# darnstrom/daqp

Measured on AMD Instinct MI355X. Metric: QPs/sec (fp64) for batched random dense QPs n=50 m=150, higher is better.
Workload: dtype f64; 1 GPU; C2: 100000 random dense QPs per GPU, n=50 m=150 ms=0, 20 active at the optimum; batch_per_gpu=100000, parallelism=1 rank(s), shards only, no data-path collective

## Files before the change

daqp_amd/_lib.py:

```python
import ctypes as C
import os
import shutil
import subprocess

PKG = os.path.dirname(os.path.abspath(__file__))
ROOT = os.path.dirname(PKG)
CSRC = os.path.join(PKG, "csrc")
LIBDIR = os.path.join(PKG, "lib")
LIBPATH = os.path.join(LIBDIR, "libdaqp_amd.so")

c_double_p = C.POINTER(C.c_double)
c_int_p = C.POINTER(C.c_int)


class DAQPSettings(C.Structure):
    _fields_ = [("primal_tol", C.c_double), ("dual_tol", C.c_double), ("zero_tol", C.c_double),
                ("pivot_tol", C.c_double), ("progress_tol", C.c_double),
                ("cycle_tol", C.c_int), ("iter_limit", C.c_int),
                ("fval_bound", C.c_double), ("eps_prox", C.c_double), ("eta_prox", C.c_double),
                ("rho_soft", C.c_double), ("rel_subopt", C.c_double), ("abs_subopt", C.c_double),
                ("sing_tol", C.c_double), ("refactor_tol", C.c_double), ("time_limit", C.c_double)]


class DAQPProblem(C.Structure):
# ... 3 lines not shown
                ("break_points", c_int_p), ("nh", C.c_int), ("problem_type", C.c_int)]


class DAQPResult(C.Structure):
    _fields_ = [("x", c_double_p), ("lam", c_double_p), ("fval", C.c_double), ("soft_slack", C.c_double),
                ("exitflag", C.c_int), ("iter", C.c_int), ("nodes", C.c_int),
                ("solve_time", C.c_double), ("setup_time", C.c_double)]


class DAQPBatchProblem(C.Structure):
    _fields_ = [("N", C.c_int), ("n", C.c_int), ("m", C.c_int), ("ms", C.c_int),
                ("H", C.c_void_p), ("f", C.c_void_p), ("A", C.c_void_p),
                ("bupper", C.c_void_p), ("blower", C.c_void_p), ("sense", C.c_void_p),
                ("memory", C.c_int)]


class DAQPBatchResult(C.Structure):
    _fields_ = [("x", C.c_void_p), ("lam", C.c_void_p), ("fval", C.c_void_p), ("soft_slack", C.c_void_p),
                ("exitflag", C.c_void_p), ("iter", C.c_void_p), ("memory", C.c_int),
                ("setup_time", C.c_double), ("solve_time", C.c_double)]


WORKSPACE_BYTES = 288
MEM_HOST, MEM_DEVICE = 0, 1

EXPORTS = [
    "daqp_quadprog", "daqp_solve", "setup_daqp", "setup_daqp_main", "daqp_update_ldp", "daqp_default_settings",
    "allocate_daqp_settings", "free_daqp_workspace", "free_daqp_ldp", "daqp_primal_init_active",
    "daqp_dual_init_active", "daqp_set_primal_start", "daqp_minrep", "allocate_daqp_workspace", "allocate_daqp_ldp", "daqp_first_violating", "daqp_batch_create", "daqp_batch_free", "daqp_amd_release_pool", "daqp_amd_shutdown", "daqp_batch_set_stream",
    "daqp_batch_set_settings", "daqp_batch_set_exact", "daqp_batch_setup", "daqp_batch_setup_shared", "daqp_batch_update", "daqp_batch_solve",
    "daqp_batch_setup_flags", "daqp_batch_working_sets", "daqp_batch_set_primal_start", "daqp_batch_prox_info", "daqp_quadprog_batch", "daqp_quadprog_batch_multi", "daqp_batch_kernel_ms",
    "daqp_batch_create_multi", "daqp_batch_free_multi", "daqp_batch_multi_shards", "daqp_batch_multi_shard", "daqp_batch_setup_multi", "daqp_batch_update_multi",
    "daqp_batch_solve_multi", "daqp_batch_setup_multi_shards", "daqp_batch_update_multi_shards", "daqp_batch_solve_multi_shards",
    "daqp_batch_device_bytes", "daqp_batch_rechecked", "daqp_batch_set_recheck", "daqp_batch_recheck_ms", "daqp_amd_last_error", "daqp_amd_device_count", "daqp_amd_version", "daqp_amd_has_tiny",
    "setup_daqp_ldp", "daqp_ldp", "ldp2qp_solution", "daqp_extract_result",
    "daqp_minrep_batch", "daqp_minrep_batch_info", "daqp_batch_reset", "reset_daqp_workspace", "daqp_deactivate_constraints",
    "daqp_batch_backward",
    "daqp_batch_enable_trace", "daqp_batch_read_trace", "daqp_batch_enable_profile", "daqp_batch_read_profile", "daqp_batch_read_ldp",
]


UNITS = {
    "daqp_amd.hip": ["daqp_amd.hip", "kernels.hip.h", "wave_ldp.hip.h", "wave_ldp_reg.hip.h", "setup_fast.hip.h", "prox.hip.h",
                     "wg_layout.hip.h", "batch_dev.hip.h", "recheck.hip.h", "minrep.hip.h", "backward.hip.h", "setup_m.hip.h", "setup_fact.hip.h", "reg_kernel.hip.h", "tiny_setup.hip.h", "setup_blk.hip.h", "multi.hip.h"],
    "reg_kernel.hip": ["reg_kernel.hip", "reg_kernel.hip.h", "wave_ldp_reg.hip.h", "wave_ldp.hip.h", "batch_dev.hip.h"],
    "reg32_kernel.hip": ["reg32_kernel.hip", "reg_kernel.hip.h", "wave_ldp_reg.hip.h", "wave_ldp.hip.h", "batch_dev.hip.h"],
    "wg_kernel.hip": ["wg_kernel.hip", "wg_kernel.hip.h", "wg_ldp.hip.h", "wg_layout.hip.h", "batch_dev.hip.h", "wave_ldp.hip.h", "wave_ldp_reg.hip.h"],
    "backward_kernel.hip": ["backward_kernel.hip", "backward.hip.h", "batch_dev.hip.h", "wave_ldp.hip.h"],
    "setup_kernel.hip": ["setup_kernel.hip", "setup_blk.hip.h", "setup_fast.hip.h", "setup_m.hip.h", "setup_fact.hip.h", "tiny_setup.hip.h", "wave_ldp_reg.hip.h", "wave_ldp.hip.h", "batch_dev.hip.h"],
}
HIPFLAGS = ["--offload-arch=gfx950", "-O3", "-std=c++17", "-ffp-contract=off", "-fPIC"]
OBJDIR = os.path.join(LIBDIR, "obj")
UNITS = {u: d for u, d in UNITS.items() if os.path.exists(os.path.join(CSRC, u))}


def units(extra_flags=()):
    return list(UNITS)


def _flag_key(extra_flags=()):
    return " ".join([*HIPFLAGS, *extra_flags])


def _unit_stale(unit, extra_flags=()):
    obj = os.path.join(OBJDIR, unit + ".o")
    if not os.path.exists(obj) or not os.path.exists(obj + ".resources.txt"):
        return True
# ... 85 lines not shown
        cur = None
        with open(path) as fh:
            for line in fh:
                m = re.search(r"remark:\s+Function Name: (\S+)", line)
                if m:
                    cur = out.setdefault(m.group(1), {})
                    continue
                m = re.search(r"remark:\s+([A-Za-z][^:]*): (\d+)", line)
                if m and cur is not None and m.group(1) in keys:
                    cur[keys[m.group(1)]] = int(m.group(2))
    try:
        names = subprocess.run(["c++filt"], input="\n".join(out), capture_output=True, text=True, check=True).stdout.split("\n")
        out = {n.replace("daqp_amd::", "").split("(")[0].replace("void ", ""): v for n, v in zip(names, out.values())}
    except (OSError, subprocess.CalledProcessError):
        pass
    return out


_lib = None


def lib():
    global _lib
    if _lib is not None:
        return _lib
    if not os.path.exists(LIBPATH):
        build()
    L = C.CDLL(os.environ.get("DAQP_AMD_LIBRARY") or LIBPATH)
    vp, ci = C.c_void_p, C.c_int
    L.daqp_amd_last_error.restype = C.c_char_p
    L.daqp_amd_version.restype = C.c_char_p
    L.daqp_batch_create.argtypes = [C.POINTER(vp), ci, ci, ci, ci, ci, C.POINTER(DAQPSettings), ci]
    L.daqp_batch_free.argtypes = [vp]
    L.daqp_batch_free.restype = None
    L.daqp_amd_release_pool.argtypes = []
    L.daqp_amd_release_pool.restype = None
    L.daqp_batch_set_stream.argtypes = [vp, vp]
    L.daqp_batch_set_stream.restype = None
    L.daqp_batch_set_settings.argtypes = [vp, C.POINTER(DAQPSettings)]
    L.daqp_batch_set_settings.restype = None
    L.daqp_batch_set_exact.argtypes = [vp, ci]
    L.daqp_batch_set_exact.restype = None
    L.daqp_batch_setup.argtypes = [vp, C.POINTER(DAQPBatchProblem), ci]
    L.daqp_batch_setup_shared.argtypes = [vp, C.POINTER(DAQPBatchProblem), ci]
    L.daqp_batch_update.argtypes = [vp, ci, C.POINTER(DAQPBatchProblem)]
    L.daqp_batch_solve.argtypes = [vp, C.POINTER(DAQPBatchResult)]
    L.daqp_batch_setup_flags.argtypes = [vp, c_int_p]
    L.daqp_batch_working_sets.argtypes = [vp, c_int_p, c_int_p]
    L.daqp_batch_set_primal_start.argtypes = [vp, C.c_void_p, ci]
    L.daqp_batch_prox_info.argtypes = [vp, c_int_p, c_int_p, C.c_void_p]
    L.daqp_quadprog_batch.argtypes = [C.POINTER(DAQPBatchResult), C.POINTER(DAQPBatchProblem), C.POINTER(DAQPSettings)]
    L.daqp_quadprog_batch_multi.argtypes = [C.POINTER(DAQPBatchResult), C.POINTER(DAQPBatchProblem), C.POINTER(DAQPSettings), c_int_p, ci]
    L.daqp_batch_create_multi.argtypes = [C.POINTER(vp), ci, ci, ci, ci, ci, C.POINTER(DAQPSettings), c_int_p, ci]
    L.daqp_batch_free_multi.argtypes = [vp]
    L.daqp_batch_free_multi.restype = None
    L.daqp_batch_multi_shards.argtypes = [vp]
    L.daqp_batch_multi_shard.argtypes = [vp, ci, c_int_p, c_int_p]
    L.daqp_batch_multi_shard.restype = vp
    L.daqp_batch_setup_multi.argtypes = [vp, C.POINTER(DAQPBatchProblem), ci]
    L.daqp_batch_update_multi.argtypes = [vp, ci, C.POINTER(DAQPBatchProblem)]
    L.daqp_batch_solve_multi.argtypes = [vp, C.POINTER(DAQPBatchResult)]
    L.daqp_batch_setup_multi_shards.argtypes = [vp, C.POINTER(DAQPBatchProblem), ci]
    L.daqp_batch_update_multi_shards.argtypes = [vp, ci, C.POINTER(DAQPBatchProblem)]
    L.daqp_batch_solve_multi_shards.argtypes = [vp, C.POINTER(DAQPBatchResult)]
    L.daqp_batch_kernel_ms.argtypes = [vp, C.POINTER(C.c_float), C.POINTER(C.c_float)]
    L.daqp_batch_rechecked.argtypes = [vp]
# ... 60 lines not shown
```

daqp_amd/csrc/daqp_amd.hip:

```cpp
#include <hip/hip_runtime.h>

#include <sched.h>

#include <chrono>
#include <cstdarg>
#include <cstdio>
#include <cstdlib>
#include <cstring>
#include <mutex>
#include <atomic>
#include <vector>
#include <string>
#include <thread>

#include "kernels.hip.h"
#include "reg_kernel.hip.h"
#include "setup_fast.hip.h"
#include "prox.hip.h"
#include "recheck.hip.h"
#include "setup_m.hip.h"
#include "setup_fact.hip.h"
#include "wg_layout.hip.h"
#include "tiny_setup.hip.h"
#include "setup_blk.hip.h"
// ... 757 lines not shown
    return k;
}
void destroy_batch(DAQPBatch *b)
{
    (void)hipSetDevice(b->device);
    (void)hipStreamSynchronize(b->stream);
    if (b->redo) { b->redo->stream = nullptr; destroy_batch(b->redo); b->redo = nullptr; }
    if (b->pin_redo) (void)hipHostFree(b->pin_redo);
    if (b->img_ho_pin) (void)hipHostFree(b->img_ho_pin);
    for (void *p : b->owned) (void)hipFree(p);
    if (b->pin_in) (void)hipHostFree(b->pin_in);
    if (b->pin_out) (void)hipHostFree(b->pin_out);
    if (b->pin_mir) (void)hipHostFree(b->pin_mir);
    if (b->pin_sig) (void)hipHostFree(b->pin_sig);
    if (b->pin_upd) (void)hipHostFree(b->pin_upd);
    if (b->ev_in) (void)hipEventDestroy(b->ev_in);
    if (b->ev_count) (void)hipEventDestroy(b->ev_count);
    if (b->pin_count) (void)hipHostFree(b->pin_count);
    for (auto &e : b->ev) if (e) (void)hipEventDestroy(e);
    for (auto &e : b->ev_r) if (e) (void)hipEventDestroy(e);
    delete b;
}
}

extern "C" {

const char *daqp_amd_last_error(void) { return g_err; }
#ifdef DAQP_AMD_FEW_VARIANTS
const char *daqp_amd_version(void) { return "daqp_amd 0.4 (gfx950, fp64: one wavefront per QP, one workgroup per QP beyond 64 working-set rows, up to 512 rows) [dev build: few template instantiations]"; }
#else
const char *daqp_amd_version(void) { return "daqp_amd 0.4 (gfx950, fp64: one wavefront per QP, one workgroup per QP beyond 64 working-set rows, up to 512 rows)"; }
#endif
int daqp_amd_has_tiny(void) { return 0; }
int daqp_amd_device_count(void)
{
    int c = 0;
    if (hipGetDeviceCount(&c) != hipSuccess) return 0;
    return c;
}
void daqp_default_settings(DAQPSettings *settings) { default_settings(settings); }

static int batch_create(DAQPBatch **out, int N, int n, int m, int ms, int ns_max, const DAQPSettings *settings, int device, int group);
int daqp_batch_create(DAQPBatch **out, int N, int n, int m, int ms, int ns_max, const DAQPSettings *settings, int device)
{
    return batch_create(out, N, n, m, ms, ns_max, settings, device, 0);
}
static int batch_create(DAQPBatch **out, int N, int n, int m, int ms, int ns_max, const DAQPSettings *settings, int device, int group)
{
    if (!out) return DAQP_EXIT_UNSUPPORTED;
    *out = nullptr;
    if (N <= 0 || n <= 0 || m < 0 || ms < 0 || ms > m || ms > n || ns_max < 0) {
        set_err("bad dimensions N=%d n=%d m=%d ms=%d ns=%d", N, n, m, ms, ns_max);
        return DAQP_EXIT_UNSUPPORTED;
    }
    const int cap = n + ns_max + 1;
    if (cap > 512 || n > 511) { set_err("n + ns + 1 = %d exceeds the 512-row working-set limit of this build", cap); return DAQP_EXIT_UNSUPPORTED; }
    int ndev = 0;
    const hipError_t dev_rc = hipGetDeviceCount(&ndev);
    if (dev_rc == hipSuccess && ndev > 0 && device >= 0 && device < 64) {
        static std::once_flag once;
        std::call_once(once, [] { if (!getenv("DAQP_AMD_NO_EXIT_SYNC")) atexit(daqp_amd_shutdown); });
        g_devices_used.fetch_or(1ull << device);
    }
    if (dev_rc != hipSuccess || ndev == 0) {
        set_err("no HIP device: libdaqp_amd has no CPU path");
        return DAQP_EXIT_UNSUPPORTED;
// ... 481 lines not shown
        if (p->sense) { memcpy(hp + o, p->sense, nb * sizeof(int)); d.sense_in = reinterpret_cast<const int *>(dp + o); }
        else d.sense_in = nullptr;
        HIPCHK(hipMemcpyAsync(b->dev_in, b->pin_in, bytes, hipMemcpyHostToDevice, b->stream));
        HIPCHK(hipEventRecord(b->ev_in, b->stream));
    } else {
        rc |= stage(b, p->f, p->memory, N * d.n, &b->sf, &b->nf, &d.f);
        rc |= stage(b, p->A, p->memory, N * d.mA * d.n, &b->sA, &b->nA, &d.A);
        rc |= stage(b, p->bupper, p->memory, N * d.m, &b->sbu, &b->nbu, &d.bu);
        rc |= stage(b, p->blower, p->memory, N * d.m, &b->sbl, &b->nbl, &d.bl);
        rc |= stage(b, p->sense, p->memory, N * d.m, &b->ssense, &b->nsense, &d.sense_in);
    }
    if (rc) return DAQP_EXIT_UNSUPPORTED;
    b->was_shared = false;
    const int mask = (init_mask & ~DAQP_UPDATE_eliminate) | DAQP_UPDATE_Rinv | DAQP_UPDATE_M | DAQP_UPDATE_v | DAQP_UPDATE_d | DAQP_UPDATE_sense;
    setup_kernel_t ks = b->setup_spill ? (d.n > 256 ? k_setup<true, 8> : k_setup<true>) : k_setup<false>;
    size_t lds_setup = b->lds_setup;
    if (b->fast_setup) {
        ks = pick_setup_fast(d.n, d.exact_setup == 0);
        lds_setup = (size_t)fast_lds(d.n, d.m, d.exact_setup, d.mA).total_bytes;
    }
    HIPCHK(hipFuncSetAttribute(reinterpret_cast<const void *>(ks), hipFuncAttributeMaxDynamicSharedMemorySize, (int)lds_setup));
    if (!b->quiet_setup) HIPCHK(hipEventRecord(b->ev[0], b->stream));
    b->inputs_adopted = p->memory == DAQP_MEM_DEVICE;
    if (!lp && b->tiny_setup) {
        hipLaunchKernelGGL(k_setup_tiny<4>, dim3((d.N + 15) / 16), dim3(64), 0, b->stream, d, mask);
        HIPCHK(hipGetLastError());
    } else if (!lp && b->fast_setup && (d.ms == 0 || !getenv("DAQP_AMD_NO_BLK_BOUNDS")) && d.n > 16 && d.exact_setup == 0 && blk_setup_enabled()) {
        const int NT = (d.n + 15) / 16;
        ldp_reg_kernel_t kb = nullptr;
#define DAQP_BLK_SHAPE(nt, nw, tail) \
        if (!kb && NT == nt && d.n <= nw && (tail) == (d.n - 16 * (nt - 1) <= 4)) kb = k_setup_blk<nt, nw, tail>;
        DAQP_BLK_SHAPES
#undef DAQP_BLK_SHAPE
        const size_t lds_blk = (size_t)(NT == 2 ? blk_lds<2>(d.n, d.m) : (NT == 3 ? blk_lds<3>(d.n, d.m) : blk_lds<4>(d.n, d.m))).total_bytes;
        HIPCHK(hipFuncSetAttribute(reinterpret_cast<const void *>(kb), hipFuncAttributeMaxDynamicSharedMemorySize, (int)lds_blk));
        if (push_descriptor(b)) return DAQP_EXIT_UNSUPPORTED;
        hipLaunchKernelGGL(kb, dim3(d.N), dim3(64), lds_blk, b->stream, (const BatchDev *)b->d_dev, mask);
        HIPCHK(hipGetLastError());
        hipLaunchKernelGGL(ks, dim3(d.N), dim3(64), lds_setup, b->stream, d, mask | kSetupOnlyMarked);
        HIPCHK(hipGetLastError());
    } else if (!lp) {
        BatchDev l = d;
        l.defer_m = defers_m(b, d) ? 1 : 0;
        const bool gs_now = b->setup_spill || (b->fact_gs && l.defer_m && b->fact_buf && d.setup_g && !(d.st.eps_prox > 0.0));
        if (l.defer_m) {
            ks = gs_now ? k_setup<true, 4, true> : k_setup<false, 4, true>;
            if (gs_now && !b->setup_spill) lds_setup = (size_t)setup_lds(d.n, d.m, true).total_bytes;
            HIPCHK(hipFuncSetAttribute(reinterpret_cast<const void *>(ks), hipFuncAttributeMaxDynamicSharedMemorySize, (int)lds_setup));
        }
        l.fact = nullptr;
        if (l.defer_m && gs_now && b->fact_buf && d.n <= kFactMaxN && !(d.st.eps_prox > 0.0)) {
            const size_t lds = fact_lds_bytes(d.n);
            if (hipFuncSetAttribute(reinterpret_cast<const void *>(k_fact_wg), hipFuncAttributeMaxDynamicSharedMemorySize, (int)lds) == hipSuccess) {
                l.fact = b->fact_buf;
                hipLaunchKernelGGL(k_fact_wg, dim3(d.N), dim3(512), lds, b->stream, l);
                HIPCHK(hipGetLastError());
            } else (void)hipGetLastError();
        }
        hipLaunchKernelGGL(ks, dim3(d.N), dim3(64), lds_setup, b->stream, l, mask);
        HIPCHK(hipGetLastError());
        if (l.defer_m) { if (launch_setup_m(b, l)) return DAQP_EXIT_UNSUPPORTED; }
    } else HIPCHK(hipMemsetAsync(d.qs, 0, (size_t)d.N * sizeof(QState), b->stream));
    b->reg_pending = false;
    if (b->lean && !lp) {
        b->n_prox_qps = 0;
    } else {
    rc = lp ? regularise(b, d, mask, true) : count_flagged_async(b, mask);
// ... 1013 lines not shown
```

daqp_amd/csrc/setup_blk.hip.h:

```cpp
#pragma once
#include "wave_ldp_reg.hip.h"
#include "batch_dev.hip.h"
#include "setup_fast.hip.h"

namespace daqp_amd {

typedef double blk_v4d __attribute__((ext_vector_type(4)));
typedef double blk_v2d __attribute__((ext_vector_type(2)));
#define BLK_GLOBAL(T) DAQP_GLOBAL(T)
template <class T> __device__ __forceinline__ auto blk_g(T *p) { return as_global(p); }

template <int NT> __host__ __device__ constexpr int blk_tix(int I, int J) { return I * NT - I * (I - 1) / 2 + (J - I); }
constexpr int kBlkScratch = 16 * 17;

template <int K> __device__ __forceinline__ double blk_bcast(double v) { return __builtin_amdgcn_update_dpp(0.0, v, 0x150 + K, 0xf, 0xf, true); }
__device__ __forceinline__ double blk_sum16(double v)
{
    v += dpp_f64<0xB1>(v);
    v += dpp_f64<0x4E>(v);
    v += dpp_f64<0x141>(v);
    v += dpp_f64<0x140>(v);
    return v;
}

template <int NT> __host__ __device__ constexpr int blk_scratch_doubles() { return (NT * (NT - 1) / 2 + NT - 1) * kBlkScratch; }

template <int NT>
__device__ __forceinline__ void blk_load(const double *Hs, int n, double zero_tol, blk_v4d (&T)[NT * (NT + 1) / 2], int &offd)
{
    const int lane = lane_id(), lr = lane & 15, lk = lane >> 4;
    offd = 0;
    static_for<NT>([&](auto Ic) __attribute__((always_inline)) {
        static_for<NT>([&](auto Jc) __attribute__((always_inline)) {
            constexpr int I = Ic, J = Jc;
            if constexpr (I <= J) {
#pragma unroll
                for (int r = 0; r < 4; ++r) {
                    const int i = 16 * I + lk + 4 * r, j = 16 * J + lr;
                    const bool in = i < n && j < n;
                    const double hij = Hs[in ? i * n + j : 0], hji = Hs[in ? j * n + i : 0];
                    if (in && j > i && (hij > zero_tol || hij < -zero_tol)) offd = 1;
                    T[blk_tix<NT>(I, J)][r] = in ? ((i == j) ? hij : 0.5 * (hij + hji)) : ((i == j) ? 1.0 : 0.0);
                }
            }
        });
    });
}

template <int NT>
__device__ __forceinline__ bool blk_factor(blk_v4d (&T)[NT * (NT + 1) / 2], int n, double zero_tol, blk_v4d (&X)[NT * (NT + 1) / 2], double *scr, double &pmin, double &pmax)
{
    const int lane = lane_id(), lr = lane & 15, lk = lane >> 4;
    blk_v4d V[NT];
    double dmin = DAQP_INF, dmax = 0.0, dsum = 0.0;
    static_for<NT>([&](auto Kc) __attribute__((always_inline)) {
        constexpr int K = Kc;
        double c[16];
        {
            const blk_v4d d = T[blk_tix<NT>(K, K)];
#pragma unroll
            for (int r = 0; r < 4; ++r)
#pragma unroll
                for (int g = 0; g < 4; ++g) c[4 * r + g] = __shfl(d[r], 16 * g + lr);
        }
        static_for<16>([&](auto kc) __attribute__((always_inline)) {
            constexpr int k = kc;
            const double d = blk_bcast<k>(c[k]);
            const bool real = 16 * K + k < n;
            dmin = fmin(dmin, real ? d : (double)DAQP_INF);
            dmax = fmax(dmax, real ? d : 0.0);
            dsum += d;
            const double inv = rsqrt(d);
            c[k] = (lr == k) ? inv : c[k] * inv;
            static_for<15 - k>([&](auto ii) __attribute__((always_inline)) {
                constexpr int i = k + 1 + ii;
                c[i] = __builtin_fma(-blk_bcast<i>(c[k]), c[k], c[i]);
            });
        });
// ... 17 lines not shown
                asm volatile("" : "+v"(x0), "+v"(x1), "+v"(x2), "+v"(x3));
                double v = x0;
                v = (lk == 1) ? x1 : v;
                v = (lk == 2) ? x2 : v;
                v = (lk == 3) ? x3 : v;
                V[K][r] = v;
            }
        }
        static_for<NT>([&](auto Jc) __attribute__((always_inline)) {
            constexpr int J = Jc;
            if constexpr (J > K) {
                blk_v4d acc = (blk_v4d){0.0, 0.0, 0.0, 0.0};
                const blk_v4d h = T[blk_tix<NT>(K, J)];
#pragma unroll
                for (int s = 0; s < 4; ++s) acc = __builtin_amdgcn_mfma_f64_16x16x4f64(V[K][s], h[s], acc, 0, 0, 0);
                T[blk_tix<NT>(K, J)] = acc;
            }
        });
        static_for<NT>([&](auto Ic) __attribute__((always_inline)) {
            static_for<NT>([&](auto Jc) __attribute__((always_inline)) {
                constexpr int I = Ic, J = Jc;
                if constexpr (I > K && J >= I) {
                    blk_v4d acc = T[blk_tix<NT>(I, J)];
                    const blk_v4d a = T[blk_tix<NT>(K, I)], bb = T[blk_tix<NT>(K, J)];
#pragma unroll
                    for (int s = 0; s < 4; ++s) acc = __builtin_amdgcn_mfma_f64_16x16x4f64(-a[s], bb[s], acc, 0, 0, 0);
                    T[blk_tix<NT>(I, J)] = acc;
                }
            });
        });
    });
    blk_v4d VT[NT > 1 ? NT - 1 : 1];
    if constexpr (NT > 1) {
        WSYNC();
        static_for<NT>([&](auto Ic) __attribute__((always_inline)) {
            static_for<NT>([&](auto Jc) __attribute__((always_inline)) {
                constexpr int I = Ic, J = Jc;
                if constexpr (I < J) {
                    double *sc = scr + (blk_tix<NT>(I, J) - I - 1) * kBlkScratch;
#pragma unroll
                    for (int r = 0; r < 4; ++r) sc[(lk + 4 * r) * 17 + lr] = T[blk_tix<NT>(I, J)][r];
                }
            });
            if constexpr (Ic < NT - 1) {
                double *sc = scr + (NT * (NT - 1) / 2 + Ic) * kBlkScratch;
#pragma unroll
                for (int r = 0; r < 4; ++r) sc[(lk + 4 * r) * 17 + lr] = V[Ic][r];
            }
        });
        WSYNC();
        static_for<NT>([&](auto Ic) __attribute__((always_inline)) {
            static_for<NT>([&](auto Jc) __attribute__((always_inline)) {
                constexpr int I = Ic, J = Jc;
                if constexpr (I < J) {
                    const double *sc = scr + (blk_tix<NT>(I, J) - I - 1) * kBlkScratch;
#pragma unroll
                    for (int s_ = 0; s_ < 4; ++s_) T[blk_tix<NT>(I, J)][s_] = sc[lr * 17 + 4 * s_ + lk];
                }
            });
            if constexpr (Ic < NT - 1) {
                const double *sc = scr + (NT * (NT - 1) / 2 + Ic) * kBlkScratch;
#pragma unroll
                for (int s_ = 0; s_ < 4; ++s_) VT[Ic][s_] = sc[lr * 17 + 4 * s_ + lk];
            }
        });
    }
    static_for<NT>([&](auto Jc) __attribute__((always_inline)) {
        constexpr int J = Jc;
        X[blk_tix<NT>(J, J)] = V[J];
        static_for<J>([&](auto Ii) __attribute__((always_inline)) {
            constexpr int I = J - 1 - Ii;
            blk_v4d s4 = (blk_v4d){0.0, 0.0, 0.0, 0.0};
            static_for<J - I>([&](auto Kk) __attribute__((always_inline)) {
                constexpr int K = I + 1 + Kk;
                const blk_v4d at = T[blk_tix<NT>(I, K)], xb = X[blk_tix<NT>(K, J)];
#pragma unroll
                for (int s_ = 0; s_ < 4; ++s_) s4 = __builtin_amdgcn_mfma_f64_16x16x4f64(at[s_], xb[s_], s4, 0, 0, 0);
            });
            blk_v4d o4 = (blk_v4d){0.0, 0.0, 0.0, 0.0};
#pragma unroll
            for (int s_ = 0; s_ < 4; ++s_) o4 = __builtin_amdgcn_mfma_f64_16x16x4f64(-VT[I][s_], s4[s_], o4, 0, 0, 0);
            X[blk_tix<NT>(I, J)] = o4;
        });
    });
    pmin = rl(dmin, 0); pmax = rl(dmax, 0);
    const double ds0 = rl(dsum, 0);
    const bool ok = (ds0 == ds0) && (pmin > 2.0 * zero_tol);
    return ok;
}

__host__ __device__ inline int blk_region(int n, int scratch) { const int h = n * n + 8; return h > scratch ? h : scratch; }
__host__ __device__ inline int blk_tile_rows(int n, int scratch)
{
    const int ldr = n | 1;
    int tr = 64;
    while (tr > 16 && tr * ldr > blk_region(n, scratch)) tr -= 16;
    return tr;
}
struct BlkLds { int R, fv, vv, xu, sens, total_bytes; };
template <int NT>
__host__ __device__ inline BlkLds blk_lds(int n, int m)
{
    BlkLds s;
    const int ldr = n | 1, TR = blk_tile_rows(n, blk_scratch_doubles<NT>());
    int r0 = blk_region(n, blk_scratch_doubles<NT>());
    if (r0 < TR * ldr) r0 = TR * ldr;
    int o = round_up(r0, 2);
    s.R = 0;
    s.fv = o; o += 64; s.vv = o; o += 64; s.xu = o; o += 64;
    s.sens = o;
    s.total_bytes = o * 8 + round_up(m, 4) * 4;
    return s;
}

template <int NT, int NW = 16 * NT, bool TAIL = false>
__global__ __launch_bounds__(64) __attribute__((amdgpu_waves_per_eu(2, 2))) void k_setup_blk(const BatchDev *__restrict__ bp, int mask)
{
    extern __shared__ __attribute__((aligned(16))) double smem[];
    static_assert(NW <= 16 * NT && NW > 16 * (NT - 1) && NW % 8 == 0, "column width within the last block");
    static_assert(!TAIL || (NT > 1 && NW == 16 * (NT - 1) + 8), "tail columns: the first eight of the last block");
    constexpr int NTT = NT * (NT + 1) / 2, KT = TAIL ? 4 * (NT - 1) + 1 : NW / 4, CT = TAIL ? NT - 1 : NT;
    const BatchDev &b = *bp;
    const int q = blockIdx.x, lane = lane_id(), lr = lane & 15, lk = lane >> 4;
    const int n = b.n, m = b.m, mA = b.mA, ms = b.ms;
    const BlkLds o = blk_lds<NT>(n, m);
    const int TR = blk_tile_rows(n, blk_scratch_doubles<NT>());
    double *Hs = smem + o.R, *fl = smem + o.fv, *vv = smem + o.vv, *xu = smem + o.xu, *tile = smem + o.R;
    double *srow = fl, *drow = vv;
    const int tailc = TAIL ? n - 16 * (NT - 1) : 0;
    int *sens = reinterpret_cast<int *>(smem + o.sens);
    const double *H = b.H + (size_t)q * n * n, *A = b.A + (size_t)q * mA * n;
    BLK_GLOBAL(QState) *qs = blk_g(b.qs + q);
    const double zero_tol = b.st.zero_tol, primal_tol = b.st.primal_tol;
    const bool force = b.st.eps_prox > 0.0;
    const bool direct = !(n & 1) && (n & 31) && !(((size_t)H | (size_t)A) & 15);
    const int ldr = direct ? n : (n | 1);
    int flag = 1, activate = 0;
    long long pt[10] = {0, 0, 0, 0, 0, 0, 0, 0, 0, 0};
    long long t0 = (kProfile && b.prof) ? (long long)__builtin_readcyclecounter() : 0;
#define SPROF(slot) do { if (kProfile && b.prof) { const long long t1 = (long long)__builtin_readcyclecounter(); pt[slot] += t1 - t0; t0 = t1; } } while (0)

    if (direct) copy_async(Hs, H, n * n);
    {
        const BLK_GLOBAL(double) *bu = blk_g(b.bu + (size_t)q * m), *bl = blk_g(b.bl + (size_t)q * m);
        const BLK_GLOBAL(int) *sin = b.sense_in ? blk_g(b.sense_in + (size_t)q * m) : nullptr;
        int bad = 0;
        for (int i = lane; i < m; i += 64) {
            int s = sin ? sin[i] : 0;
            if (s & DAQP_BINARY) bad |= 2;
            if (!(s & DAQP_IMMUTABLE)) {
                const double diff = bu[i] - bl[i];
                if (diff < -primal_tol) bad |= 1;
                else if (diff < zero_tol && !(s & DAQP_SOFT)) { s |= DAQP_ACTIVE + DAQP_IMMUTABLE; bad |= 4; }
            }
            sens[i] = s;
        }
        bad = (__any(bad & 2) ? 2 : 0) | (__any(bad & 1) ? 1 : 0) | (__any(bad & 4) ? 4 : 0);
        if (b.sense_in) activate = 1;
        if (bad & 4) activate = 1;
        if (bad & 2) flag = DAQP_EXIT_UNSUPPORTED;
        else if (bad & 1) flag = DAQP_EXIT_INFEASIBLE;
        if (force && flag > 0) flag = DAQP_NEEDS_SHIFT;
        fl[lane] = (lane < n) ? blk_g(b.f)[(size_t)q * n + lane] : 0.0;
    }
    int diag = 0;
    blk_v4d X[NTT];
    if (flag > 0) {
        if (direct) copy_wait(); else stage_rows(Hs, H, n, n, n);
        WSYNC();
        blk_v4d T[NTT];
        int offd;
        blk_load<NT>(Hs, n, zero_tol, T, offd);
        SPROF(9);
        if (!__any(offd) && ms > 0) flag = DAQP_NEEDS_ORDERED;
        else if (!__any(offd)) {
            const double hd = (lane < n) ? Hs[lane * n + lane] : 1.0;
            const double ha = hd < 0 ? -hd : hd;
            const double hscale = -wave_min((lane < n) ? -ha : 0.0);
            const double ftol = hscale > 0 ? zero_tol * hscale : zero_tol;
            const bool fail = lane < n && hd <= ftol;
            const int code = (b.st.eps_prox == 0.0 && hd <= zero_tol) ? DAQP_EXIT_NONCONVEX : DAQP_NEEDS_SHIFT;
            const unsigned long long fm = __ballot(fail);
            if (fm) flag = __builtin_amdgcn_readlane(code, __ffsll((long long)fm) - 1);
            else {
                WSYNC();
                xu[lane] = 1 / sqrt(hd);
                WSYNC();
                static_for<NT>([&](auto Ic) __attribute__((always_inline)) {
                    static_for<NT>([&](auto Jc) __attribute__((always_inline)) {
                        constexpr int I = Ic, J = Jc;
                        if constexpr (I <= J) {
#pragma unroll
                            for (int r = 0; r < 4; ++r) X[blk_tix<NT>(I, J)][r] = (I == J && lk + 4 * r == lr) ? xu[16 * I + lr] : 0.0;
                        }
                    });
                });
                diag = 1;
            }
            WSYNC();
        } else {
            WSYNC();
            double pmin = DAQP_INF, pmax = 0.0;
            const bool ok = blk_factor<NT>(T, n, zero_tol, X, Hs, pmin, pmax);
            if (!ok || !(pmin > 2.0 * zero_tol * pmax)) flag = DAQP_NEEDS_ORDERED;
            WSYNC();
        }
    }
    if (flag == DAQP_NEEDS_ORDERED) { if (lane == 0) qs->setup_flag = DAQP_NEEDS_ORDERED; return; }
    SPROF(0);
    int unc = 0;
    double vcol[NT];
    static_for<NT>([&](auto Jc) __attribute__((always_inline)) { vcol[Jc] = 0.0; });
    if (flag > 0) {
        static_for<NT>([&](auto Jc) __attribute__((always_inline)) {
            constexpr int J = Jc;
            double p = 0;
            static_for<J + 1>([&](auto Ic) __attribute__((always_inline)) {
#pragma unroll
                for (int r = 0; r < 4; ++r) p = __builtin_fma(X[blk_tix<NT>(Ic, J)][r], fl[16 * Ic + lk + 4 * r], p);
            });
            p += __shfl_xor(p, 16);
            p += __shfl_xor(p, 32);
            vcol[J] = p;
            if (lk == 0 && 16 * J + lr < n) blk_g(b.v)[(size_t)q * n + 16 * J + lr] = p;
        });
        SPROF(1);
        if (mask & DAQP_UPDATE_unconstrained) {
            int fixed = 0;
            for (int i = lane; i < m; i += 64) fixed |= sens[i] & (DAQP_ACTIVE + DAQP_IMMUTABLE);
            if (!__any(fixed)) {
                unc = 1;
                static_for<NT>([&](auto Ic) __attribute__((always_inline)) {
                    constexpr int I = Ic;
#pragma unroll
                    for (int r = 0; r < 4; ++r) {
                        double p = 0;
                        static_for<NT - I>([&](auto Jj) __attribute__((always_inline)) { p = __builtin_fma(X[blk_tix<NT>(I, I + Jj)][r], vcol[I + Jj], p); });
                        p = blk_sum16(p);
                        if (lr == 0) xu[16 * I + lk + 4 * r] = -p;
                    }
                });
// ... 210 lines not shown
#pragma unroll
                            for (int u = 0; u < 8; ++u) dst[(size_t)((tq + u < npair) ? tq + u : npair - 1) * 64] = (blk_v2d){v8[u].x * scal, v8[u].y * scal};
                        }
                    } else {
                        for (int tq = 0; tq < npair; tq += 8) {
                            double vx[8], vy[8];
#pragma unroll
                            for (int u = 0; u < 8; ++u) {
                                const int t = (tq + u < npair) ? tq + u : npair - 1;
                                vx[u] = a[2 * t];
                                const double y = a[(2 * t + 1 < n) ? 2 * t + 1 : 2 * t];
                                vy[u] = (2 * t + 1 < n) ? y : 0.0;
                            }
#pragma unroll
                            for (int u = 0; u < 8; ++u) dst[(size_t)((tq + u < npair) ? tq + u : npair - 1) * 64] = (blk_v2d){vx[u] * scal, vy[u] * scal};
                        }
                    }
                }
            }
            if (direct && tb + TR < mA) {
                WSYNC();
                copy_async(tile, A + (size_t)(tb + TR) * n, ((mA - tb - TR) < TR ? (mA - tb - TR) : TR) * n);
            }
            if (__any(rowbad)) flag = DAQP_EXIT_INFEASIBLE;
            SPROF(4);
        }
    }
    const int all_feasible = __all(feasible);
    int sing = kEmpty;
    if (flag > 0 && unc && all_feasible) { sing = DAQP_UNCONSTRAINED_OPTIMAL; activate = 0; }
    if (flag > 0) {
        if (lane < n && unc) blk_g(b.xunc)[(size_t)q * n + lane] = xu[lane];
    }
    for (int i = lane; i < m; i += 64) blk_g(b.sense)[(size_t)q * m + i] = sens[i];
    SPROF(5);
    if (lane == 0) {
        qs->n_active = 0; qs->reuse_ind = 0; qs->sing_ind = sing; qs->iterations = 0;
        qs->lam_swapped = 0; qs->setup_flag = flag; qs->need_activate = (flag > 0) ? activate : 0; qs->pad_ = 0;
        qs->exitflag = flag; qs->fval = 0; qs->soft_slack = 0; qs->diag_h = diag; qs->n_prox = 0;
        qs->upd_flag = 0;
        if (kProfile && b.prof) for (int i = 0; i < 10; ++i) blk_g(b.prof)[(size_t)q * 32 + i] = pt[i];
    }
#undef SPROF
}

#define DAQP_BLK_SHAPES \
    DAQP_BLK_SHAPE(2, 24, true) DAQP_BLK_SHAPE(2, 32, false) DAQP_BLK_SHAPE(3, 40, true) DAQP_BLK_SHAPE(3, 48, false) \
    DAQP_BLK_SHAPE(4, 56, true) DAQP_BLK_SHAPE(4, 56, false) DAQP_BLK_SHAPE(4, 64, false)

}
```

include/daqp_amd.h:

```cpp
#ifndef DAQP_AMD_H
#define DAQP_AMD_H

#ifdef __cplusplus
extern "C" {
#endif

typedef double c_float;

#define DAQP_EXIT_SOFT_OPTIMAL 2
#define DAQP_EXIT_OPTIMAL 1
#define DAQP_EXIT_INFEASIBLE -1
#define DAQP_EXIT_CYCLE -2
#define DAQP_EXIT_UNBOUNDED -3
#define DAQP_EXIT_ITERLIMIT -4
#define DAQP_EXIT_NONCONVEX -5
#define DAQP_EXIT_OVERDETERMINED_INITIAL -6
#define DAQP_EXIT_TIMELIMIT -7
#define DAQP_EXIT_UNSUPPORTED -8
#define DAQP_BACKWARD_SINGULAR -20

#define DAQP_UPDATE_Rinv 1
#define DAQP_UPDATE_M 2
#define DAQP_UPDATE_v 4
#define DAQP_UPDATE_d 8
// ... 133 lines not shown
int daqp_quadprog_batch(DAQPBatchResult *r, const DAQPBatchProblem *p, const DAQPSettings *settings);

typedef struct DAQPMultiBatch DAQPMultiBatch;
int daqp_batch_create_multi(DAQPMultiBatch **out, int N, int n, int m, int ms, int ns_max, const DAQPSettings *settings,
                            const int *devices, int n_devices);
void daqp_batch_free_multi(DAQPMultiBatch *mb);
int daqp_batch_multi_shards(const DAQPMultiBatch *mb);
DAQPBatch *daqp_batch_multi_shard(DAQPMultiBatch *mb, int g, int *shard_N, int *device);
int daqp_batch_setup_multi(DAQPMultiBatch *mb, const DAQPBatchProblem *p, int init_mask);
int daqp_batch_update_multi(DAQPMultiBatch *mb, int mask, const DAQPBatchProblem *p);
int daqp_batch_solve_multi(DAQPMultiBatch *mb, DAQPBatchResult *r);
int daqp_batch_setup_multi_shards(DAQPMultiBatch *mb, const DAQPBatchProblem *ps , int init_mask);
int daqp_batch_update_multi_shards(DAQPMultiBatch *mb, int mask, const DAQPBatchProblem *ps );
int daqp_batch_solve_multi_shards(DAQPMultiBatch *mb, DAQPBatchResult *rs );
int daqp_quadprog_batch_multi(DAQPBatchResult *r, const DAQPBatchProblem *p, const DAQPSettings *settings,
                              const int *devices, int n_devices);

int daqp_batch_kernel_ms(DAQPBatch *b, float *setup_ms, float *solve_ms);
int daqp_batch_rechecked(const DAQPBatch *b);
void daqp_batch_set_recheck(DAQPBatch *b, int on);
int daqp_batch_recheck_ms(DAQPBatch *b, float *ms);
unsigned long long daqp_batch_device_bytes(const DAQPBatch *b);

int daqp_batch_enable_trace(DAQPBatch *b, int cap);
int daqp_batch_read_trace(DAQPBatch *b, int *host );
int daqp_batch_enable_profile(DAQPBatch *b, int on);
int daqp_batch_read_profile(DAQPBatch *b, long long *host );
int daqp_batch_read_ldp(DAQPBatch *b, int q, c_float *M, c_float *R, c_float *v, c_float *dupper, c_float *dlower, c_float *scaling);

const char *daqp_amd_last_error(void);
int daqp_amd_device_count(void);
const char *daqp_amd_version(void);
int daqp_amd_has_tiny(void);

#ifdef __cplusplus
}
#endif
#endif
```

Baseline: 4.162 million QPs/s.

## Stream Hessian in 16-row bands to shrink block setup LDS footprint

The block-setup kernel no longer stages the full n×n Hessian in LDS. It loads it in 16-row bands through a two-band ping-pong buffer with async copies, and splits the transpose scratch into two trips for NT>=4. The LDS size is now sized toward a target of about 20 KB, which lets more workgroups fit on each CU. In exchange the load adds extra wave syncs and a global read for the diagonal check, and a query API for the LDS layout is exposed.

Result: no change. 4.162 million QPs/s, median of 2 (+0.0%).

```diff
diff --git a/daqp_amd/_lib.py b/daqp_amd/_lib.py
--- a/daqp_amd/_lib.py
+++ b/daqp_amd/_lib.py
@@ -59,7 +59,7 @@
     "daqp_batch_setup_flags", "daqp_batch_working_sets", "daqp_batch_set_primal_start", "daqp_batch_prox_info", "daqp_quadprog_batch", "daqp_quadprog_batch_multi", "daqp_batch_kernel_ms",
     "daqp_batch_create_multi", "daqp_batch_free_multi", "daqp_batch_multi_shards", "daqp_batch_multi_shard", "daqp_batch_setup_multi", "daqp_batch_update_multi",
     "daqp_batch_solve_multi", "daqp_batch_setup_multi_shards", "daqp_batch_update_multi_shards", "daqp_batch_solve_multi_shards",
-    "daqp_batch_device_bytes", "daqp_batch_rechecked", "daqp_batch_set_recheck", "daqp_batch_recheck_ms", "daqp_amd_last_error", "daqp_amd_device_count", "daqp_amd_version", "daqp_amd_has_tiny",
+    "daqp_batch_device_bytes", "daqp_batch_rechecked", "daqp_batch_set_recheck", "daqp_batch_recheck_ms", "daqp_amd_last_error", "daqp_amd_device_count", "daqp_amd_version", "daqp_amd_has_tiny", "daqp_amd_setup_blk_lds",
     "setup_daqp_ldp", "daqp_ldp", "ldp2qp_solution", "daqp_extract_result",
     "daqp_minrep_batch", "daqp_minrep_batch_info", "daqp_batch_reset", "reset_daqp_workspace", "daqp_deactivate_constraints",
     "daqp_batch_backward",
@@ -211,6 +211,8 @@
     L.daqp_amd_version.restype = C.c_char_p
     L.daqp_batch_create.argtypes = [C.POINTER(vp), ci, ci, ci, ci, ci, C.POINTER(DAQPSettings), ci]
     L.daqp_batch_free.argtypes = [vp]
+    if hasattr(L, "daqp_amd_setup_blk_lds"):
+        L.daqp_amd_setup_blk_lds.argtypes = [ci, ci, ci, c_int_p]
     L.daqp_batch_free.restype = None
     L.daqp_amd_release_pool.argtypes = []
     L.daqp_amd_release_pool.restype = None
diff --git a/daqp_amd/csrc/daqp_amd.hip b/daqp_amd/csrc/daqp_amd.hip
--- a/daqp_amd/csrc/daqp_amd.hip
+++ b/daqp_amd/csrc/daqp_amd.hip
@@ -813,6 +813,13 @@
 const char *daqp_amd_version(void) { return "daqp_amd 0.4 (gfx950, fp64: one wavefront per QP, one workgroup per QP beyond 64 working-set rows, up to 512 rows)"; }
 #endif
 int daqp_amd_has_tiny(void) { return 0; }
+int daqp_amd_setup_blk_lds(int n, int m, int ms, int *tile_rows)
+{
+    if (n <= 16 || n > 64 || m < 0 || ms < 0 || ms > n) return -1;
+    const BlkLds o = blk_lds_any(n, m, ms);
+    if (tile_rows) *tile_rows = o.TR;
+    return o.total_bytes;
+}
 int daqp_amd_device_count(void)
 {
     int c = 0;
@@ -1360,7 +1367,7 @@
         if (!kb && NT == nt && d.n <= nw && (tail) == (d.n - 16 * (nt - 1) <= 4)) kb = k_setup_blk<nt, nw, tail>;
         DAQP_BLK_SHAPES
 #undef DAQP_BLK_SHAPE
-        const size_t lds_blk = (size_t)(NT == 2 ? blk_lds<2>(d.n, d.m) : (NT == 3 ? blk_lds<3>(d.n, d.m) : blk_lds<4>(d.n, d.m))).total_bytes;
+        const size_t lds_blk = (size_t)blk_lds_any(d.n, d.m, d.ms).total_bytes;
         HIPCHK(hipFuncSetAttribute(reinterpret_cast<const void *>(kb), hipFuncAttributeMaxDynamicSharedMemorySize, (int)lds_blk));
         if (push_descriptor(b)) return DAQP_EXIT_UNSUPPORTED;
         hipLaunchKernelGGL(kb, dim3(d.N), dim3(64), lds_blk, b->stream, (const BatchDev *)b->d_dev, mask);
diff --git a/daqp_amd/csrc/setup_blk.hip.h b/daqp_amd/csrc/setup_blk.hip.h
--- a/daqp_amd/csrc/setup_blk.hip.h
+++ b/daqp_amd/csrc/setup_blk.hip.h
@@ -23,7 +23,9 @@
     return v;
 }
 
-template <int NT> __host__ __device__ constexpr int blk_scratch_doubles() { return (NT * (NT - 1) / 2 + NT - 1) * kBlkScratch; }
+template <int NT> __host__ __device__ constexpr int blk_slots() { return NT * (NT - 1) / 2 + NT - 1; }
+template <int NT> __host__ __device__ constexpr int blk_trip_slots() { return NT >= 4 ? (blk_slots<NT>() + 1) / 2 : blk_slots<NT>(); }
+template <int NT> __host__ __device__ constexpr int blk_scratch_doubles() { return blk_trip_slots<NT>() * kBlkScratch; }
 
 template <int NT>
 __device__ __forceinline__ void blk_load(const double *Hs, int n, double zero_tol, blk_v4d (&T)[NT * (NT + 1) / 2], int &offd)
@@ -44,6 +46,35 @@
                 }
             }
         });
+    });
+}
+
+template <int NT, int B>
+__device__ __forceinline__ void blk_load_band(const double *Hb, int n, double zero_tol, blk_v4d (&T)[NT * (NT + 1) / 2], int &offd)
+{
+    const int lane = lane_id(), lr = lane & 15, lk = lane >> 4;
+    static_for<NT>([&](auto Jc) __attribute__((always_inline)) {
+        constexpr int J = Jc;
+        if constexpr (J >= B) {
+#pragma unroll
+            for (int r = 0; r < 4; ++r) {
+                const int i = 16 * B + lk + 4 * r, j = 16 * J + lr;
+                const bool in = i < n && j < n;
+                const double hij = Hb[in ? (lk + 4 * r) * n + j : 0];
+                if (in && j > i && (hij > zero_tol || hij < -zero_tol)) offd = 1;
+                T[blk_tix<NT>(B, J)][r] = hij;
+            }
+        }
+    });
+    static_for<B + 1>([&](auto Ic) __attribute__((always_inline)) {
+        constexpr int I = Ic;
+#pragma unroll
+        for (int r = 0; r < 4; ++r) {
+            const int i = 16 * I + lk + 4 * r, j = 16 * B + lr;
+            const bool in = i < n && j < n;
+            const double hij = T[blk_tix<NT>(I, B)][r], hji = Hb[in ? lr * n + i : 0];
+            T[blk_tix<NT>(I, B)][r] = in ? ((i == j) ? hij : 0.5 * (hij + hji)) : ((i == j) ? 1.0 : 0.0);
+        }
     });
 }
 
@@ -127,37 +158,53 @@
     });
     blk_v4d VT[NT > 1 ? NT - 1 : 1];
     if constexpr (NT > 1) {
-        WSYNC();
-        static_for<NT>([&](auto Ic) __attribute__((always_inline)) {
-            static_for<NT>([&](auto Jc) __attribute__((always_inline)) {
-                constexpr int I = Ic, J = Jc;
-                if constexpr (I < J) {
-                    double *sc = scr + (blk_tix<NT>(I, J) - I - 1) * kBlkScratch;
-#pragma unroll
-                    for (int r = 0; r < 4; ++r) sc[(lk + 4 * r) * 17 + lr] = T[blk_tix<NT>(I, J)][r];
-                }
-            });
-            if constexpr (Ic < NT - 1) {
-                double *sc = scr + (NT * (NT - 1) / 2 + Ic) * kBlkScratch;
-#pragma unroll
-                for (int r = 0; r < 4; ++r) sc[(lk + 4 * r) * 17 + lr] = V[Ic][r];
-            }
-        });
-        WSYNC();
-        static_for<NT>([&](auto Ic) __attribute__((always_inline)) {
-            static_for<NT>([&](auto Jc) __attribute__((always_inline)) {
-                constexpr int I = Ic, J = Jc;
-                if constexpr (I < J) {
-                    const double *sc = scr + (blk_tix<NT>(I, J) - I - 1) * kBlkScratch;
-#pragma unroll
-                    for (int s_ = 0; s_ < 4; ++s_) T[blk_tix<NT>(I, J)][s_] = sc[lr * 17 + 4 * s_ + lk];
-                }
-            });
-            if constexpr (Ic < NT - 1) {
-                const double *sc = scr + (NT * (NT - 1) / 2 + Ic) * kBlkScratch;
-#pragma unroll
-                for (int s_ = 0; s_ < 4; ++s_) VT[Ic][s_] = sc[lr * 17 + 4 * s_ + lk];
-            }
+        constexpr int TS = blk_trip_slots<NT>(), TRIPS = (blk_slots<NT>() + TS - 1) / TS;
+        static_for<TRIPS>([&](auto Pc) __attribute__((always_inline)) {
+            constexpr int P = Pc;
+            WSYNC();
+            static_for<NT>([&](auto Ic) __attribute__((always_inline)) {
+                static_for<NT>([&](auto Jc) __attribute__((always_inline)) {
+                    constexpr int I = Ic, J = Jc;
+                    if constexpr (I < J) {
+                        constexpr int slot = blk_tix<NT>(I, J) - I - 1;
+                        if constexpr (slot / TS == P) {
+                            double *sc = scr + (slot % TS) * kBlkScratch;
+#pragma unroll
+                            for (int r = 0; r < 4; ++r) sc[(lk + 4 * r) * 17 + lr] = T[blk_tix<NT>(I, J)][r];
+                        }
+                    }
+                });
+                if constexpr (Ic < NT - 1) {
+                    constexpr int slot = NT * (NT - 1) / 2 + Ic;
+                    if constexpr (slot / TS == P) {
+                        double *sc = scr + (slot % TS) * kBlkScratch;
+#pragma unroll
+                        for (int r = 0; r < 4; ++r) sc[(lk + 4 * r) * 17 + lr] = V[Ic][r];
+                    }
+                }
+            });
+            WSYNC();
+            static_for<NT>([&](auto Ic) __attribute__((always_inline)) {
+                static_for<NT>([&](auto Jc) __attribute__((always_inline)) {
+                    constexpr int I = Ic, J = Jc;
+                    if constexpr (I < J) {
+                        constexpr int slot = blk_tix<NT>(I, J) - I - 1;
+                        if constexpr (slot / TS == P) {
+                            const double *sc = scr + (slot % TS) * kBlkScratch;
+#pragma unroll
+                            for (int s_ = 0; s_ < 4; ++s_) T[blk_tix<NT>(I, J)][s_] = sc[lr * 17 + 4 * s_ + lk];
+                        }
+                    }
+                });
+                if constexpr (Ic < NT - 1) {
+                    constexpr int slot = NT * (NT - 1) / 2 + Ic;
+                    if constexpr (slot / TS == P) {
+                        const double *sc = scr + (slot % TS) * kBlkScratch;
+#pragma unroll
+                        for (int s_ = 0; s_ < 4; ++s_) VT[Ic][s_] = sc[lr * 17 + 4 * s_ + lk];
+                    }
+                }
+            });
         });
     }
     static_for<NT>([&](auto Jc) __attribute__((always_inline)) {
@@ -184,28 +231,34 @@
     return ok;
 }
 
-__host__ __device__ inline int blk_region(int n, int scratch) { const int h = n * n + 8; return h > scratch ? h : scratch; }
-__host__ __device__ inline int blk_tile_rows(int n, int scratch)
-{
-    const int ldr = n | 1;
-    int tr = 64;
-    while (tr > 16 && tr * ldr > blk_region(n, scratch)) tr -= 16;
-    return tr;
-}
-struct BlkLds { int R, fv, vv, xu, sens, total_bytes; };
+constexpr int kBlkLdsTarget = 20480;
+struct BlkLds { int R, fv, vv, xu, sens, total_bytes, TR; };
 template <int NT>
-__host__ __device__ inline BlkLds blk_lds(int n, int m)
+__host__ __device__ inline BlkLds blk_lds(int n, int m, int ms)
 {
     BlkLds s;
-    const int ldr = n | 1, TR = blk_tile_rows(n, blk_scratch_doubles<NT>());
-    int r0 = blk_region(n, blk_scratch_doubles<NT>());
-    if (r0 < TR * ldr) r0 = TR * ldr;
+    const int ldr = n | 1, behind = 3 * 64 * 8 + round_up(m, 4) * 4;
+    int need = (n < 32 ? n : 32) * n;
+    if (need < blk_scratch_doubles<NT>()) need = blk_scratch_doubles<NT>();
+    if (ms > 0 && need < n * n + 8) need = n * n + 8;
+    const int fits = (kBlkLdsTarget - behind) / 8;
+    const int cap = need > fits ? need : fits;
+    int tr = 64;
+    while (tr > 16 && tr * ldr > cap) tr -= 16;
+    s.TR = tr;
+    int r0 = need;
+    if (r0 < tr * ldr) r0 = tr * ldr;
     int o = round_up(r0, 2);
     s.R = 0;
     s.fv = o; o += 64; s.vv = o; o += 64; s.xu = o; o += 64;
     s.sens = o;
     s.total_bytes = o * 8 + round_up(m, 4) * 4;
     return s;
+}
+__host__ __device__ inline BlkLds blk_lds_any(int n, int m, int ms)
+{
+    const int NT = (n + 15) / 16;
+    return NT == 2 ? blk_lds<2>(n, m, ms) : (NT == 3 ? blk_lds<3>(n, m, ms) : blk_lds<4>(n, m, ms));
 }
 
 template <int NT, int NW = 16 * NT, bool TAIL = false>
@@ -218,8 +271,8 @@
     const BatchDev &b = *bp;
     const int q = blockIdx.x, lane = lane_id(), lr = lane & 15, lk = lane >> 4;
     const int n = b.n, m = b.m, mA = b.mA, ms = b.ms;
-    const BlkLds o = blk_lds<NT>(n, m);
-    const int TR = blk_tile_rows(n, blk_scratch_doubles<NT>());
+    const BlkLds o = blk_lds<NT>(n, m, ms);
+    const int TR = o.TR;
     double *Hs = smem + o.R, *fl = smem + o.fv, *vv = smem + o.vv, *xu = smem + o.xu, *tile = smem + o.R;
     double *srow = fl, *drow = vv;
     const int tailc = TAIL ? n - 16 * (NT - 1) : 0;
@@ -235,7 +288,8 @@
     long long t0 = (kProfile && b.prof) ? (long long)__builtin_readcyclecounter() : 0;
 #define SPROF(slot) do { if (kProfile && b.prof) { const long long t1 = (long long)__builtin_readcyclecounter(); pt[slot] += t1 - t0; t0 = t1; } } while (0)
 
-    if (direct) copy_async(Hs, H, n * n);
+    const int bandd = 16 * n;
+    if (direct) { copy_async(Hs, H, bandd); copy_async(Hs + bandd, H + bandd, (n < 32 ? n - 16 : 16) * n); }
     {
         const BLK_GLOBAL(double) *bu = blk_g(b.bu + (size_t)q * m), *bl = blk_g(b.bl + (size_t)q * m);
         const BLK_GLOBAL(int) *sin = b.sense_in ? blk_g(b.sense_in + (size_t)q * m) : nullptr;
@@ -261,15 +315,25 @@
     int diag = 0;
     blk_v4d X[NTT];
     if (flag > 0) {
-        if (direct) copy_wait(); else stage_rows(Hs, H, n, n, n);
-        WSYNC();
         blk_v4d T[NTT];
-        int offd;
-        blk_load<NT>(Hs, n, zero_tol, T, offd);
+        int offd = 0;
+        static_for<NT>([&](auto Bc) __attribute__((always_inline)) {
+            constexpr int B = Bc;
+            double *Hb = Hs + (B & 1) * bandd;
+            if constexpr (B % 2 == 0) {
+                if (direct) copy_wait();
+                else { WSYNC(); stage_rows(Hb, H + (size_t)B * bandd, (n - 16 * B < 32) ? n - 16 * B : 32, n, n); }
+            }
+            WSYNC();
+            blk_load_band<NT, B>(Hb, n, zero_tol, T, offd);
+            if constexpr (B + 2 < NT) {
+                if (direct) { WSYNC(); copy_async(Hb, H + (size_t)(B + 2) * bandd, ((n - 16 * (B + 2) < 16) ? n - 16 * (B + 2) : 16) * n); }
+            }
+        });
         SPROF(9);
         if (!__any(offd) && ms > 0) flag = DAQP_NEEDS_ORDERED;
         else if (!__any(offd)) {
-            const double hd = (lane < n) ? Hs[lane * n + lane] : 1.0;
+            const double hd = (lane < n) ? blk_g(b.H)[(size_t)q * n * n + lane * n + lane] : 1.0;
             const double ha = hd < 0 ? -hd : hd;
             const double hscale = -wave_min((lane < n) ? -ha : 0.0);
             const double ftol = hscale > 0 ? zero_tol * hscale : zero_tol;
diff --git a/include/daqp_amd.h b/include/daqp_amd.h
--- a/include/daqp_amd.h
+++ b/include/daqp_amd.h
@@ -189,6 +189,7 @@
 int daqp_amd_device_count(void);
 const char *daqp_amd_version(void);
 int daqp_amd_has_tiny(void);
+int daqp_amd_setup_blk_lds(int n, int m, int ms, int *tile_rows);
 
 #ifdef __cplusplus
 }
```

## Shrink blocked-setup LDS footprint with XOR-swizzled scratch and byte-sized sense

Applied to the files above, without the earlier changes.

Replaces the padded 17-stride transpose scratch with a 16-stride XOR swizzle, stores constraint sense flags as bytes in LDS, overlaps the f vector region with the H/tile region by keeping f in a register until factorization finishes, and sizes tile rows against an occupancy-oriented LDS budget (one eighth of 160KB). The aim is to cut LDS per workgroup so more QP workgroups can be resident per CU. It adds extra sync and a merge of upper sense bits from sense_in on writeback, and the tile sizing logic now depends on m and ms.

Measured after the change: 4.188 million QPs/s before, 4.216 million QPs/s after, median of 6. About the same (+0.7%).

```diff
diff --git a/daqp_amd/csrc/daqp_amd.hip b/daqp_amd/csrc/daqp_amd.hip
--- a/daqp_amd/csrc/daqp_amd.hip
+++ b/daqp_amd/csrc/daqp_amd.hip
@@ -1360,7 +1360,7 @@
         if (!kb && NT == nt && d.n <= nw && (tail) == (d.n - 16 * (nt - 1) <= 4)) kb = k_setup_blk<nt, nw, tail>;
         DAQP_BLK_SHAPES
 #undef DAQP_BLK_SHAPE
-        const size_t lds_blk = (size_t)(NT == 2 ? blk_lds<2>(d.n, d.m) : (NT == 3 ? blk_lds<3>(d.n, d.m) : blk_lds<4>(d.n, d.m))).total_bytes;
+        const size_t lds_blk = (size_t)(NT == 2 ? blk_lds<2>(d.n, d.m, d.ms) : (NT == 3 ? blk_lds<3>(d.n, d.m, d.ms) : blk_lds<4>(d.n, d.m, d.ms))).total_bytes;
         HIPCHK(hipFuncSetAttribute(reinterpret_cast<const void *>(kb), hipFuncAttributeMaxDynamicSharedMemorySize, (int)lds_blk));
         if (push_descriptor(b)) return DAQP_EXIT_UNSUPPORTED;
         hipLaunchKernelGGL(kb, dim3(d.N), dim3(64), lds_blk, b->stream, (const BatchDev *)b->d_dev, mask);
diff --git a/daqp_amd/csrc/setup_blk.hip.h b/daqp_amd/csrc/setup_blk.hip.h
--- a/daqp_amd/csrc/setup_blk.hip.h
+++ b/daqp_amd/csrc/setup_blk.hip.h
@@ -11,7 +11,7 @@
 template <class T> __device__ __forceinline__ auto blk_g(T *p) { return as_global(p); }
 
 template <int NT> __host__ __device__ constexpr int blk_tix(int I, int J) { return I * NT - I * (I - 1) / 2 + (J - I); }
-constexpr int kBlkScratch = 16 * 17;
+constexpr int kBlkScratch = 16 * 16;
 
 template <int K> __device__ __forceinline__ double blk_bcast(double v) { return __builtin_amdgcn_update_dpp(0.0, v, 0x150 + K, 0xf, 0xf, true); }
 __device__ __forceinline__ double blk_sum16(double v)
@@ -134,13 +134,13 @@
                 if constexpr (I < J) {
                     double *sc = scr + (blk_tix<NT>(I, J) - I - 1) * kBlkScratch;
 #pragma unroll
-                    for (int r = 0; r < 4; ++r) sc[(lk + 4 * r) * 17 + lr] = T[blk_tix<NT>(I, J)][r];
+                    for (int r = 0; r < 4; ++r) sc[(lk + 4 * r) * 16 + (lr ^ (lk + 4 * r))] = T[blk_tix<NT>(I, J)][r];
                 }
             });
             if constexpr (Ic < NT - 1) {
                 double *sc = scr + (NT * (NT - 1) / 2 + Ic) * kBlkScratch;
 #pragma unroll
-                for (int r = 0; r < 4; ++r) sc[(lk + 4 * r) * 17 + lr] = V[Ic][r];
+                for (int r = 0; r < 4; ++r) sc[(lk + 4 * r) * 16 + (lr ^ (lk + 4 * r))] = V[Ic][r];
             }
         });
         WSYNC();
@@ -150,13 +150,13 @@
                 if constexpr (I < J) {
                     const double *sc = scr + (blk_tix<NT>(I, J) - I - 1) * kBlkScratch;
 #pragma unroll
-                    for (int s_ = 0; s_ < 4; ++s_) T[blk_tix<NT>(I, J)][s_] = sc[lr * 17 + 4 * s_ + lk];
+                    for (int s_ = 0; s_ < 4; ++s_) T[blk_tix<NT>(I, J)][s_] = sc[lr * 16 + ((4 * s_ + lk) ^ lr)];
                 }
             });
             if constexpr (Ic < NT - 1) {
                 const double *sc = scr + (NT * (NT - 1) / 2 + Ic) * kBlkScratch;
 #pragma unroll
-                for (int s_ = 0; s_ < 4; ++s_) VT[Ic][s_] = sc[lr * 17 + 4 * s_ + lk];
+                for (int s_ = 0; s_ < 4; ++s_) VT[Ic][s_] = sc[lr * 16 + ((4 * s_ + lk) ^ lr)];
             }
         });
     }
@@ -184,27 +184,34 @@
     return ok;
 }
 
-__host__ __device__ inline int blk_region(int n, int scratch) { const int h = n * n + 8; return h > scratch ? h : scratch; }
-__host__ __device__ inline int blk_tile_rows(int n, int scratch)
+constexpr int kBlkLdsEighth = 160 * 1024 / 8, kBlkVecs = 3 * 64;
+__host__ __device__ inline int blk_region(int n, int ms, int scratch)
 {
-    const int ldr = n | 1;
+    int h = n * n + 8 - kBlkVecs;
+    if (ms > 0 && h < n * n) h = n * n;
+    return h > scratch ? h : scratch;
+}
+__host__ __device__ inline int blk_tile_rows(int n, int m, int ms, int scratch)
+{
+    const int ldr = n | 1, eighth = (kBlkLdsEighth - round_up(m, 8)) / 8 - kBlkVecs;
+    const int cap = blk_region(n, ms, scratch) > eighth ? blk_region(n, ms, scratch) : eighth;
     int tr = 64;
-    while (tr > 16 && tr * ldr > blk_region(n, scratch)) tr -= 16;
+    while (tr > 16 && tr * ldr > cap) tr -= 16;
     return tr;
 }
 struct BlkLds { int R, fv, vv, xu, sens, total_bytes; };
 template <int NT>
-__host__ __device__ inline BlkLds blk_lds(int n, int m)
+__host__ __device__ inline BlkLds blk_lds(int n, int m, int ms)
 {
     BlkLds s;
-    const int ldr = n | 1, TR = blk_tile_rows(n, blk_scratch_doubles<NT>());
-    int r0 = blk_region(n, blk_scratch_doubles<NT>());
+    const int ldr = n | 1, TR = blk_tile_rows(n, m, ms, blk_scratch_doubles<NT>());
+    int r0 = blk_region(n, ms, blk_scratch_doubles<NT>());
     if (r0 < TR * ldr) r0 = TR * ldr;
     int o = round_up(r0, 2);
     s.R = 0;
     s.fv = o; o += 64; s.vv = o; o += 64; s.xu = o; o += 64;
     s.sens = o;
-    s.total_bytes = o * 8 + round_up(m, 4) * 4;
+    s.total_bytes = o * 8 + round_up(m, 8);
     return s;
 }
 
@@ -218,12 +225,12 @@
     const BatchDev &b = *bp;
     const int q = blockIdx.x, lane = lane_id(), lr = lane & 15, lk = lane >> 4;
     const int n = b.n, m = b.m, mA = b.mA, ms = b.ms;
-    const BlkLds o = blk_lds<NT>(n, m);
-    const int TR = blk_tile_rows(n, blk_scratch_doubles<NT>());
+    const BlkLds o = blk_lds<NT>(n, m, ms);
+    const int TR = blk_tile_rows(n, m, ms, blk_scratch_doubles<NT>());
     double *Hs = smem + o.R, *fl = smem + o.fv, *vv = smem + o.vv, *xu = smem + o.xu, *tile = smem + o.R;
     double *srow = fl, *drow = vv;
     const int tailc = TAIL ? n - 16 * (NT - 1) : 0;
-    int *sens = reinterpret_cast<int *>(smem + o.sens);
+    unsigned char *sens = reinterpret_cast<unsigned char *>(smem + o.sens);
     const double *H = b.H + (size_t)q * n * n, *A = b.A + (size_t)q * mA * n;
     BLK_GLOBAL(QState) *qs = blk_g(b.qs + q);
     const double zero_tol = b.st.zero_tol, primal_tol = b.st.primal_tol;
@@ -231,6 +238,7 @@
     const bool direct = !(n & 1) && (n & 31) && !(((size_t)H | (size_t)A) & 15);
     const int ldr = direct ? n : (n | 1);
     int flag = 1, activate = 0;
+    double f_lane = 0.0;
     long long pt[10] = {0, 0, 0, 0, 0, 0, 0, 0, 0, 0};
     long long t0 = (kProfile && b.prof) ? (long long)__builtin_readcyclecounter() : 0;
 #define SPROF(slot) do { if (kProfile && b.prof) { const long long t1 = (long long)__builtin_readcyclecounter(); pt[slot] += t1 - t0; t0 = t1; } } while (0)
@@ -248,7 +256,7 @@
                 if (diff < -primal_tol) bad |= 1;
                 else if (diff < zero_tol && !(s & DAQP_SOFT)) { s |= DAQP_ACTIVE + DAQP_IMMUTABLE; bad |= 4; }
             }
-            sens[i] = s;
+            sens[i] = (unsigned char)s;
         }
         bad = (__any(bad & 2) ? 2 : 0) | (__any(bad & 1) ? 1 : 0) | (__any(bad & 4) ? 4 : 0);
         if (b.sense_in) activate = 1;
@@ -256,7 +264,7 @@
         if (bad & 2) flag = DAQP_EXIT_UNSUPPORTED;
         else if (bad & 1) flag = DAQP_EXIT_INFEASIBLE;
         if (force && flag > 0) flag = DAQP_NEEDS_SHIFT;
-        fl[lane] = (lane < n) ? blk_g(b.f)[(size_t)q * n + lane] : 0.0;
+        if (lane < n) f_lane = blk_g(b.f)[(size_t)q * n + lane];
     }
     int diag = 0;
     blk_v4d X[NTT];
@@ -302,6 +310,9 @@
         }
     }
     if (flag == DAQP_NEEDS_ORDERED) { if (lane == 0) qs->setup_flag = DAQP_NEEDS_ORDERED; return; }
+    if (direct && flag <= 0) copy_wait();
+    fl[lane] = f_lane;
+    WSYNC();
     SPROF(0);
     int unc = 0;
     double vcol[NT];
@@ -578,7 +589,7 @@
     if (flag > 0) {
         if (lane < n && unc) blk_g(b.xunc)[(size_t)q * n + lane] = xu[lane];
     }
-    for (int i = lane; i < m; i += 64) blk_g(b.sense)[(size_t)q * m + i] = sens[i];
+    for (int i = lane; i < m; i += 64) blk_g(b.sense)[(size_t)q * m + i] = (b.sense_in ? blk_g(b.sense_in)[(size_t)q * m + i] & ~0xff : 0) | sens[i];
     SPROF(5);
     if (lane == 0) {
         qs->n_active = 0; qs->reuse_ind = 0; qs->sing_ind = sing; qs->iterations = 0;
```
